# VITA-Group/Open-L2O

Measured on NVIDIA H100. Metric: coordinate-updates/sec (N_params x unroll_steps), higher is better.
Workload: dtype f32

## Files before the change

open_l2o_b200/csrc/cwlstm_tc.cuh:

```cuda
#pragma once
#include "cwlstm_common.cuh"
#include "l2o_internal.h"

namespace l2o {
namespace tc {

constexpr int kH = 20;
constexpr int kN = 4 * kH;
constexpr int kTile = 64;
constexpr int kU = 5;
constexpr int kFwdWG = 3;
constexpr int kFwdThreads = 128 * kFwdWG;
template <int N>
struct IC {
  static constexpr int value = N;
};

template <class C>
struct Geo {
  static constexpr bool FC = C::FC;
  static constexpr int ColH1 = FC ? 24 : 4, ColH2 = FC ? 44 : 24;
  static constexpr int ColOne = FC ? 20 : C::F;
  static constexpr int KB = FC ? 8 : 6;
  static constexpr int L1Lo = 0, L1Hi = FC ? 6 : 3;
  static constexpr int L2Lo = FC ? 2 : 0, L2Hi = KB;
  static constexpr int K1 = 8 * (L1Hi - L1Lo), K2 = 8 * (L2Hi - L2Lo);
  static constexpr int N1 = FC ? 48 : 24, N2 = 48;
  static constexpr int B1Floats = K1 * kN, B2Floats = K2 * kN, T1Floats = kN * N1, T2Floats = kN * N2;
  static constexpr int FwdFloats = 2 * (B1Floats + B2Floats);
  static constexpr int AllFloats = FwdFloats + 2 * (T1Floats + T2Floats);
  static_assert(!FC || C::F == 20, "fc preprocessing: dim 20");
  static_assert(FC || C::F <= 3, "feature chunk: at most 3 features");
};
constexpr int kImgMaxFloats = Geo<Cfg<L2O_PRE_FC, 2, 20, 20, 20>>::AllFloats;

__device__ __forceinline__ uint32_t smem_u32(const void* p) { return (uint32_t)__cvta_generic_to_shared(p); }

__device__ __forceinline__ void mbar_init(uint64_t* bar, uint32_t count) {
  asm volatile("mbarrier.init.shared::cta.b64 [%0], %1;" ::"r"(smem_u32(bar)), "r"(count));
}
__device__ __forceinline__ void mbar_expect_tx(uint64_t* bar, uint32_t bytes) {
  asm volatile("mbarrier.arrive.expect_tx.shared::cta.b64 _, [%0], %1;" ::"r"(smem_u32(bar)), "r"(bytes) : "memory");
}
__device__ __forceinline__ void mbar_wait(uint64_t* bar, uint32_t parity) {
  asm volatile(
      "{\n\t"
      ".reg .pred p;\n\t"
      "WAIT_LOOP:\n\t"
      "mbarrier.try_wait.parity.shared::cta.b64 p, [%0], %1;\n\t"
      "@p bra WAIT_DONE;\n\t"
      "bra WAIT_LOOP;\n\t"
      "WAIT_DONE:\n\t"
      "}\n" ::"r"(smem_u32(bar)),
      "r"(parity)
      : "memory");
}
__device__ __forceinline__ void fence_barrier_init() { asm volatile("fence.mbarrier_init.release.cluster;" ::: "memory"); }
__device__ __forceinline__ void fence_proxy_async() { asm volatile("fence.proxy.async.shared::cta;" ::: "memory"); }
__device__ __forceinline__ void tma_bulk_g2s(void* dst, const void* src, uint32_t bytes, uint64_t* bar) {
  asm volatile("cp.async.bulk.shared::cluster.global.mbarrier::complete_tx::bytes [%0], [%1], %2, [%3];" ::"r"(
                   smem_u32(dst)),
               "l"(src), "r"(bytes), "r"(smem_u32(bar))
               : "memory");
}
__device__ __forceinline__ void stage_image(float* dst, const float* src, uint32_t bytes, uint64_t* bar) {
  if (threadIdx.x == 0) {
    mbar_expect_tx(bar, bytes);
    tma_bulk_g2s(dst, src, bytes, bar);
  }
  mbar_wait(bar, 0);
}

__device__ __forceinline__ void wg_fence() { asm volatile("wgmma.fence.sync.aligned;" ::: "memory"); }
__device__ __forceinline__ void wg_commit() { asm volatile("wgmma.commit_group.sync.aligned;" ::: "memory"); }
template <int N>
__device__ __forceinline__ void wg_wait() {
  asm volatile("wgmma.wait_group.sync.aligned %0;" ::"n"(N) : "memory");
}

__device__ __forceinline__ uint64_t make_desc(uint32_t saddr, uint32_t lbo, uint32_t sbo) {
  return (uint64_t)((saddr & 0x3FFFFu) >> 4) | ((uint64_t)(lbo >> 4) << 16) | ((uint64_t)(sbo >> 4) << 32);
}
__device__ __forceinline__ uint64_t img_desc(const float* p, int ncols) {
  return make_desc(smem_u32(p), (uint32_t)(ncols / 8) * 128u, 128u);
}
__host__ __device__ constexpr uint64_t img_kstep(int ncols) { return (uint64_t)((2 * (ncols / 8) * 128) >> 4); }

#define L2O_ACC8(b) "+f"(d[b]), "+f"(d[b + 1]), "+f"(d[b + 2]), "+f"(d[b + 3]), "+f"(d[b + 4]), "+f"(d[b + 5]), \
                    "+f"(d[b + 6]), "+f"(d[b + 7])
__device__ __forceinline__ void mma_rs_n80(float* d, const uint32_t* a, uint64_t b, uint32_t acc) {
  asm volatile(
      "{\n\t.reg .pred p;\n\tsetp.ne.b32 p, %45, 0;\n\t"
      "wgmma.mma_async.sync.aligned.m64n80k8.f32.tf32.tf32 "
      "{%0,%1,%2,%3,%4,%5,%6,%7,%8,%9,%10,%11,%12,%13,%14,%15,%16,%17,%18,%19,"
      "%20,%21,%22,%23,%24,%25,%26,%27,%28,%29,%30,%31,%32,%33,%34,%35,%36,%37,%38,%39}, "
      "{%40,%41,%42,%43}, %44, p, 1, 1;\n\t}\n"
      : L2O_ACC8(0), L2O_ACC8(8), L2O_ACC8(16), L2O_ACC8(24), L2O_ACC8(32)
      : "r"(a[0]), "r"(a[1]), "r"(a[2]), "r"(a[3]), "l"(b), "r"(acc));
}
__device__ __forceinline__ void mma_rs_n48(float* d, const uint32_t* a, uint64_t b, uint32_t acc) {
  asm volatile(
      "{\n\t.reg .pred p;\n\tsetp.ne.b32 p, %29, 0;\n\t"
      "wgmma.mma_async.sync.aligned.m64n48k8.f32.tf32.tf32 "
      "{%0,%1,%2,%3,%4,%5,%6,%7,%8,%9,%10,%11,%12,%13,%14,%15,%16,%17,%18,%19,%20,%21,%22,%23}, "
      "{%24,%25,%26,%27}, %28, p, 1, 1;\n\t}\n"
      : L2O_ACC8(0), L2O_ACC8(8), L2O_ACC8(16)
      : "r"(a[0]), "r"(a[1]), "r"(a[2]), "r"(a[3]), "l"(b), "r"(acc));
}
__device__ __forceinline__ void mma_rs_n24(float* d, const uint32_t* a, uint64_t b, uint32_t acc) {
  asm volatile(
      "{\n\t.reg .pred p;\n\tsetp.ne.b32 p, %17, 0;\n\t"
      "wgmma.mma_async.sync.aligned.m64n24k8.f32.tf32.tf32 "
      "{%0,%1,%2,%3,%4,%5,%6,%7,%8,%9,%10,%11}, "
      "{%12,%13,%14,%15}, %16, p, 1, 1;\n\t}\n"
      : L2O_ACC8(0), "+f"(d[8]), "+f"(d[9]), "+f"(d[10]), "+f"(d[11])
      : "r"(a[0]), "r"(a[1]), "r"(a[2]), "r"(a[3]), "l"(b), "r"(acc));
}
template <int N>
__device__ __forceinline__ void mma_rs(float* d, const uint32_t* a, uint64_t b, uint32_t acc) {
  static_assert(N == 80 || N == 48 || N == 24, "wgmma width");
  if constexpr (N == 80) mma_rs_n80(d, a, b, acc);
  else if constexpr (N == 48) mma_rs_n48(d, a, b, acc);
  else mma_rs_n24(d, a, b, acc);
}

__device__ __forceinline__ float to_tf32(float x) {
  uint32_t r;
  asm("cvt.rna.tf32.f32 %0, %1;" : "=r"(r) : "f"(x));
  return __uint_as_float(r);
}
__device__ __forceinline__ void split_tf32(float x, uint32_t& hi, uint32_t& lo) {
  hi = __float_as_uint(x) & 0xFFFFE000u;
  lo = __float_as_uint(x - __uint_as_float(hi));
}

__host__ __device__ constexpr int vec_unit(int c, int base) { return 5 * ((c - base) & 3) + ((c - base) >> 2); }
__host__ __device__ constexpr int unit_col(int u, int base) { return base + 4 * (u % 5) + u / 5; }
__host__ __device__ constexpr int gate_ref_col(int n) {
  return (2 * ((n >> 3) & 1) + (n & 1)) * kH + 5 * ((n & 7) >> 1) + (n >> 4);
}
__host__ __device__ constexpr int dx_gate_col(int k) { return (k & ~7) + 2 * (k & 3) + ((k >> 2) & 1); }
__host__ __device__ constexpr int dx_group(int c) { return c / 24; }
__host__ __device__ constexpr int dx_unit(int c) {
  return 2 * ((c % 24) >> 3) + (c & 1) >= 5 ? -1 : 5 * ((c & 7) >> 1) + 2 * ((c % 24) >> 3) + (c & 1);
}
__host__ __device__ constexpr int img_index(int k, int n, int ncols) {
  return ((k >> 2) * (ncols / 8) + (n >> 3)) * 32 + (n & 7) * 4 + (k & 3);
}

template <class C>
__device__ __forceinline__ float ext_weight(const float* __restrict__ theta, bool l2, int c, int n) {
  using G = Geo<C>;
  const int col = gate_ref_col(n);
  if (c == G::ColOne) return theta[(l2 ? C::O_B2 : C::O_B1) + col];
  const bool in_h1 = c >= G::ColH1 && c < G::ColH1 + kH, in_h2 = c >= G::ColH2 && c < G::ColH2 + kH;
  if (!l2) {
    if (in_h1) return theta[C::O_W1 + (C::F + vec_unit(c, G::ColH1)) * C::G1 + col];
    if (G::FC && c < kH) return theta[C::O_W1 + vec_unit(c, 0) * C::G1 + col];
    if (!G::FC && c < C::F) return theta[C::O_W1 + c * C::G1 + col];
    return 0.f;
  }
  if (in_h1) return theta[C::O_W2 + vec_unit(c, G::ColH1) * C::G2 + col];
  if (in_h2) return theta[C::O_W2 + (kH + vec_unit(c, G::ColH2)) * C::G2 + col];
  return 0.f;
}
constexpr float kLog2e = 1.4426950408889634f;
__host__ __device__ constexpr float gate_scale(int gate) { return gate == 1 ? -2.f * kLog2e : -kLog2e; }
constexpr int kGateF = 2;
__device__ __forceinline__ float sigmoid_scaled(float zs) { return rcp_approx(1.0f + ex2_approx(zs)); }
__device__ __forceinline__ float tanh_scaled(float zs) { return fmaf(2.0f, rcp_approx(1.0f + ex2_approx(zs)), -1.0f); }

template <class C>
__host__ __device__ constexpr int dx_operand_col(bool l2, int c) {
  using G = Geo<C>;
  return l2 ? unit_col(dx_unit(c), dx_group(c) == 0 ? G::ColH1 : G::ColH2)
            : unit_col(dx_unit(c), dx_group(c) == 0 ? G::ColH1 : 0);
}

template <class C>
__global__ void prep_weights_kernel(const float* __restrict__ theta, float* __restrict__ img, int with_transposed) {
  static_assert(C::H1 == kH && C::H2 == kH && (C::F <= 3 || C::FC), "tc engine: LSTM-20x2, F <= 3 or fc(20)");
  using G = Geo<C>;
  const int nb = (G::K1 + G::K2) * kN;
  const int nt = with_transposed ? kN * (G::N1 + G::N2) : 0;
  for (int e = blockIdx.x * blockDim.x + threadIdx.x; e < nb + nt; e += gridDim.x * blockDim.x) {
    float w;
    float* hi;
    int off, idx;
    if (e < nb) {
      const bool l2 = e >= G::K1 * kN;
      const int ee = l2 ? e - G::K1 * kN : e;
      const int k = ee / kN, n = ee % kN;
      const int c = 8 * (l2 ? G::L2Lo : G::L1Lo) + k, gate = gate_ref_col(n) / kH;
      w = ext_weight<C>(theta, l2, c, n);
      if (c == G::ColOne && gate == kGateF) w += 1.0f;
      w *= gate_scale(gate);
      hi = img + (l2 ? 2 * G::B1Floats : 0);
      off = l2 ? G::B2Floats : G::B1Floats;
      idx = img_index(k, n, kN);
    } else {
      const int e2 = e - nb;
      const bool l2 = e2 >= kN * G::N1;
      const int nc = l2 ? G::N2 : G::N1;
      const int ee = l2 ? e2 - kN * G::N1 : e2;
      const int k = ee / nc, n = ee % nc;
      w = dx_unit(n) < 0 ? 0.f : ext_weight<C>(theta, l2, dx_operand_col<C>(l2, n), dx_gate_col(k));
      hi = img + G::FwdFloats + (l2 ? 2 * G::T1Floats : 0);
      off = l2 ? G::T2Floats : G::T1Floats;
      idx = img_index(k, n, nc);
    }
    const float h = to_tf32(w);
    hi[idx] = h;
    hi[off + idx] = to_tf32(w - h);
  }
}

template <int KB>
struct Frag {
  uint32_t hi[KB][4], lo[KB][4];
  __device__ __forceinline__ void zero() {
#pragma unroll
    for (int k = 0; k < KB; ++k)
#pragma unroll
      for (int r = 0; r < 4; ++r) { hi[k][r] = 0u; lo[k][r] = 0u; }
  }
  __device__ __forceinline__ void put_at(int c, int rh, float v) {
    split_tf32(v, hi[c / 8][((c / 4) & 1) * 2 + rh], lo[c / 8][((c / 4) & 1) * 2 + rh]);
  }
  __device__ __forceinline__ float get_at(int c, int rh) const {
    return __uint_as_float(hi[c / 8][((c / 4) & 1) * 2 + rh]) + __uint_as_float(lo[c / 8][((c / 4) & 1) * 2 + rh]);
  }
  template <int COL>
  __device__ __forceinline__ void put(int rh, float v) {
    static_assert(COL % 4 == 0 && COL / 8 < KB, "fragment column");
    put_at(COL, rh, v);
  }
  template <int BASE>
  __device__ __forceinline__ void put_vec(int rh, const float* v) {
    static_assert(BASE % 4 == 0 && (BASE + 19) / 8 < KB, "fragment column");
#pragma unroll
    for (int s = 0; s < kU; ++s) put_at(BASE + 4 * s, rh, v[s]);
  }
};

template <int N, int KB, int LO, int HI>
__device__ __forceinline__ void mma3(float* d, const Frag<KB>& f, uint64_t bh, uint64_t bl) {
  constexpr uint64_t step = img_kstep(N);
#pragma unroll
  for (int kb = LO; kb < HI; ++kb) {
    const uint64_t o = (uint64_t)(kb - LO) * step;
    mma_rs<N>(d, f.lo[kb], bh + o, kb > LO ? 1u : 0u);
    mma_rs<N>(d, f.hi[kb], bl + o, 1u);
    mma_rs<N>(d, f.hi[kb], bh + o, 1u);
  }
}

__host__ __device__ constexpr int acc_idx(int s, int g, int rh) { return 4 * (2 * s + (g >> 1)) + 2 * rh + (g & 1); }

__device__ __forceinline__ void lstm_point_fwd(float zi, float zj, float zf, float zo, float& c, float& h) {
  const float Ei = ex2_approx(fminf(zi, 40.f));
  const float Ej = ex2_approx(fminf(zj, 40.f));
  const float Qf = 1.0f + ex2_approx(fminf(zf, 40.f));
  const float Pij = (1.0f + Ei) * (1.0f + Ej);
  const float cn = fmaf(c, Pij, (1.0f - Ej) * Qf) * rcp_approx(Pij * Qf);
  c = cn;
  const float Ec = ex2_approx(fminf(-2.f * kLog2e * cn, 63.f));
  const float Eo = ex2_approx(fminf(zo, 63.f));
  h = (1.0f - Ec) * rcp_approx((1.0f + Ec) * (1.0f + Eo));
}
__device__ __forceinline__ float elu_fast(float av) {
  const float em = ex2_approx(kLog2e * av) - 1.0f;
  const float ep = av * fmaf(av, fmaf(av, fmaf(av, 1.0f / 24.0f, 1.0f / 6.0f), 0.5f), 1.0f);
  return av > 0.f ? av : (av > -0.0625f ? ep : em);
}

__device__ __forceinline__ void load5(const float* __restrict__ p, int q, float* v) {
#pragma unroll
  for (int s = 0; s < kU; ++s) v[s] = p[5 * q + s];
}
__device__ __forceinline__ void store5(float* __restrict__ p, int q, const float* v) {
#pragma unroll
  for (int s = 0; s < kU; ++s) p[5 * q + s] = v[s];
}
__device__ __forceinline__ float quad_sum(float v) {
  v += __shfl_xor_sync(0xffffffffu, v, 1);
  return v + __shfl_xor_sync(0xffffffffu, v, 2);
}
__device__ __forceinline__ float from_row(float v, int lane, int rh) {
  return __shfl_sync(0xffffffffu, v, (lane & ~3) | rh);
}

struct FwdExtra {
  const int32_t* step_ptr;
  int32_t t_offset;
  float p_fixed;
};

template <class C>
struct SmemF {
  float img[Geo<C>::FwdFloats];
  float wo[kH + 4];
  float win[64];
  uint64_t wbar;
};
template <class C>
__host__ __device__ constexpr size_t adamc_offset() {
  return (sizeof(SmemF<C>) + 15) & ~(size_t)15;
}
template <class C>
__host__ __device__ constexpr size_t fwd_smem_bytes(int T) {
  return adamc_offset<C>() + (C::FC ? (size_t)T * 2 * sizeof(float) : 0);
}
__device__ __forceinline__ double warp_sum_pairs_d(double v) {
  v += __shfl_xor_sync(0xffffffffu, v, 16);
  v += __shfl_xor_sync(0xffffffffu, v, 8);
  v += __shfl_xor_sync(0xffffffffu, v, 4);
  return v + __shfl_xor_sync(0xffffffffu, v, 1);
}

template <class C, bool FAST = false, int OPT = L2O_OPT_NONE, bool CKPT = false>
__global__ void __launch_bounds__(kFwdThreads, 1) unroll_fwd_kernel(l2o_unroll_args a, NetRt rt, const float* __restrict__ img,
                                                                     float* __restrict__ state_out, FwdExtra ex) {
  static_assert(!FAST || (!C::FC && OPT != L2O_OPT_NONE), "the full-tile forward is the DM nets' with an optimizee");
  using G = Geo<C>;
  extern __shared__ __align__(128) unsigned char smem_raw[];
  SmemF<C>& S = *reinterpret_cast<SmemF<C>*>(smem_raw);
  const int T = a.T;
  const int64_t n = a.n;
  const bool in_kernel_opt = FAST || a.opt_kind != L2O_OPT_NONE;
  const int opt_kind = FAST ? OPT : a.opt_kind;
  const bool want_fx = in_kernel_opt && a.fx != nullptr;
  const bool adam_mode = C::NIN == 2 && a.m != nullptr;
  const bool has_ckpt = FAST ? CKPT : a.ckpt != nullptr;
  const bool has_grec = FAST ? CKPT : a.g_rec != nullptr;
  const bool tanh_out = !FAST && rt.tanh_output;
  const bool has_delta = !FAST && a.delta_seq != nullptr;
  const bool has_labels = !FAST && a.labels != nullptr;
  float* adamc = reinterpret_cast<float*>(smem_raw + adamc_offset<C>());

  if (threadIdx.x < kH) S.wo[threadIdx.x] = a.theta[C::O_WO + threadIdx.x];
  if (threadIdx.x == kH) S.wo[kH] = a.theta[C::O_BO];
  if constexpr (C::FC) {
    static_assert(!C::FC || C::NIN == 2, "fc nets here are RNNprop nets (two inputs)");
    if (threadIdx.x >= 32 && threadIdx.x < 92) S.win[threadIdx.x - 32] = a.theta[C::O_WIN + threadIdx.x - 32];
    if (adam_mode) {
      const int step0 = ex.step_ptr ? *ex.step_ptr + ex.t_offset : a.step0;
      for (int t = threadIdx.x; t < T; t += blockDim.x) {
        const float p = (ex.step_ptr == nullptr && ex.p_fixed > 0.f) ? ex.p_fixed : (float)(step0 + t);
        adamc[2 * t] = 1.0f - powf(a.beta1, p);
        adamc[2 * t + 1] = 1.0f - powf(a.beta2, p);
      }
    }
  }
  if (threadIdx.x == 0) {
    mbar_init(&S.wbar, 1);
    fence_barrier_init();
  }
  __syncthreads();
  stage_image(S.img, img, G::FwdFloats * 4, &S.wbar);

  const int wg = __shfl_sync(0xffffffffu, threadIdx.x >> 7, 0), warp = (threadIdx.x >> 5) & 3, lane = threadIdx.x & 31;
  const int g = lane >> 2, q = lane & 3, own = q & 1;
  const uint64_t b1h = img_desc(S.img, kN), b1l = img_desc(S.img + G::B1Floats, kN);
  const uint64_t b2h = img_desc(S.img + 2 * G::B1Floats, kN), b2l = img_desc(S.img + 2 * G::B1Floats + G::B2Floats, kN);
  const int64_t ntiles = (n + kTile - 1) / kTile;
  const int64_t slot = n * C::SF;
  const int64_t nk = n * kH;
  const float bo = S.wo[kH];
  float wo[kU];
#pragma unroll
  for (int s = 0; s < kU; ++s) wo[s] = S.wo[5 * q + s];
  double imit = 0.0;
  float d[kN / 2];
#pragma unroll
  for (int k = 0; k < kN / 2; ++k) d[k] = 0.f;

  for (int64_t tile = (int64_t)blockIdx.x * kFwdWG + wg; tile < ntiles; tile += (int64_t)gridDim.x * kFwdWG) {
    const int64_t r0 = tile * kTile + warp * 16 + g;
    const int64_t row[2] = {r0, r0 + 8};
    const bool act[2] = {FAST || row[0] < n, FAST || row[1] < n};
    const int64_t io = own ? row[1] : row[0];
    const bool oact = FAST || io < n;
    const bool writer = q < 2 && oact;
    float* ck = has_ckpt ? a.ckpt + r0 * kH : nullptr;
    float* gr = has_grec ? a.g_rec + io : nullptr;
    Frag<G::KB> A;
    A.zero();
    float c1[2][kU], c2[2][kU];
#pragma unroll
    for (int rh = 0; rh < 2; ++rh) {
      float h1[kU] = {0.f, 0.f, 0.f, 0.f, 0.f}, h2[kU] = {0.f, 0.f, 0.f, 0.f, 0.f};
#pragma unroll
      for (int s = 0; s < kU; ++s) { c1[rh][s] = 0.f; c2[rh][s] = 0.f; }
      if (act[rh]) {
        const int64_t i = row[rh];
        load5(a.state + i * kH, q, h1);
        load5(a.state + (n + i) * kH, q, c1[rh]);
        load5(a.state + 2 * n * kH + i * kH, q, h2);
        load5(a.state + 2 * n * kH + (n + i) * kH, q, c2[rh]);
        if (has_ckpt) {
          float* p = ck + rh * 8 * kH;
          store5(p, q, h1);
          store5(p + nk, q, c1[rh]);
          store5(p + 2 * nk, q, h2);
          store5(p + 3 * nk, q, c2[rh]);
        }
        if (!FAST && T == 0 && state_out != a.state) {
          store5(state_out + i * kH, q, h1);
          store5(state_out + (n + i) * kH, q, c1[rh]);
          store5(state_out + 2 * n * kH + i * kH, q, h2);
          store5(state_out + 2 * n * kH + (n + i) * kH, q, c2[rh]);
        }
      }
      A.template put_vec<G::ColH1>(rh, h1);
      A.template put_vec<G::ColH2>(rh, h2);
    }
    if constexpr (G::FC) {
      A.template put<G::ColOne>(0, q == 0 ? 1.0f : 0.f);
      A.template put<G::ColOne>(1, q == 0 ? 1.0f : 0.f);
    }
    float x = 0.f, oa = 0.f, ob = 0.f, am = 0.f, av = 0.f;
    if (oact) {
      if (FAST || a.x) x = a.x[io];
      if (in_kernel_opt) { oa = a.opt_a[io]; ob = a.opt_b[io]; }
      if (adam_mode) { am = a.m[io]; av = a.v[io]; }
    }
// ... 193 lines not shown
```

open_l2o_b200/csrc/cwlstm_tc_bwd.cuh:

```cuda
#pragma once
#include <type_traits>
#include "cwlstm_tc.cuh"

namespace l2o {
namespace tcb {

using namespace tc;

constexpr int kBwdWG = 2;
constexpr int kBwdThreads = 128 * kBwdWG;
constexpr uint32_t kXaLBO = 8 * 128;
constexpr uint32_t kXbLBO = 10 * 128;
constexpr uint32_t kXaBytes = 8 * kXaLBO;
constexpr uint32_t kXbBytes = 8 * kXbLBO;
constexpr int kBlkL1 = 5, kRowOne2 = 63;

__device__ __forceinline__ void split_bf16x2(float v0, float v1, uint32_t& hi, uint32_t& lo) {
  asm("cvt.rn.bf16x2.f32 %0, %1, %2;" : "=r"(hi) : "f"(v1), "f"(v0));
  const float r0 = v0 - __uint_as_float(hi << 16), r1 = v1 - __uint_as_float(hi & 0xFFFF0000u);
  asm("cvt.rn.bf16x2.f32 %0, %1, %2;" : "=r"(lo) : "f"(r1), "f"(r0));
}
__device__ __forceinline__ void stsm_x4_trans(uint32_t sa, uint32_t r0, uint32_t r1, uint32_t r2, uint32_t r3) {
  asm volatile("stmatrix.sync.aligned.m8n8.x4.trans.shared.b16 [%0], {%1, %2, %3, %4};" ::"r"(sa), "r"(r0), "r"(r1),
               "r"(r2), "r"(r3)
               : "memory");
}
__device__ __forceinline__ void mma_ss_bf16_n80(float* d, uint64_t a, uint64_t b) {
  asm volatile(
      "{\n\t.reg .pred p;\n\tsetp.ne.b32 p, %42, 0;\n\t"
      "wgmma.mma_async.sync.aligned.m64n80k16.f32.bf16.bf16 "
      "{%0,%1,%2,%3,%4,%5,%6,%7,%8,%9,%10,%11,%12,%13,%14,%15,%16,%17,%18,%19,"
      "%20,%21,%22,%23,%24,%25,%26,%27,%28,%29,%30,%31,%32,%33,%34,%35,%36,%37,%38,%39}, "
      "%40, %41, p, 1, 1, 0, 0;\n\t}\n"
      : L2O_ACC8(0), L2O_ACC8(8), L2O_ACC8(16), L2O_ACC8(24), L2O_ACC8(32)
      : "l"(a), "l"(b), "r"(1));
}
__device__ __forceinline__ void wg_bar(int wg) { asm volatile("bar.sync %0, 128;" ::"r"(1 + wg) : "memory"); }
__device__ __forceinline__ void prefetch_l2_bulk(const void* p, uint32_t bytes) {
  asm volatile("cp.async.bulk.prefetch.L2.global [%0], %1;" ::"l"(p), "r"(bytes) : "memory");
}
__device__ __forceinline__ void prefetch_l2(const void* p) { asm volatile("prefetch.global.L2 [%0];" ::"l"(p)); }

__device__ __forceinline__ void unit_bwd(float& zi, float& zj, float& zf, float& zo, float cprev, float dh, float& dc, float& hn) {
  const float i = sigmoid_scaled(zi), j = tanh_scaled(zj), f = sigmoid_scaled(zf), o = sigmoid_scaled(zo);
  const float cn = fmaf(f, cprev, i * j);
  const float tcn = tanh_fast(cn);
  hn = tcn * o;
  const float dho = dh * o;
  const float dcv = fmaf(dho, fmaf(-tcn, tcn, 1.0f), dc);
  zi = (dcv * j) * fmaf(-i, i, i);
  zj = (dcv * i) * fmaf(-j, j, 1.0f);
  zf = (dcv * cprev) * fmaf(-f, f, f);
  zo = (dho * tcn) * (1.0f - o);
  dc = dcv * f;
}

template <class C, int MODE>
__device__ __forceinline__ int dw_row(int m) {
  const int p = (m & 7) >> 1, slot = 2 * (m >> 3) + (m & 1);
  if (m == kRowOne2) return MODE == 2 ? C::O_B1 : C::O_B2;
  if (slot < 2 * kBlkL1) {
    const int u = 5 * p + slot % kU;
    if (MODE == 2) return C::O_W1 + (slot < kU ? C::F + u : u) * C::G1;
    return C::O_W2 + (slot < kU ? u : kH + u) * C::G2;
  }
  if (MODE == 0) {
    const int s = slot - 2 * kBlkL1;
    if (s < kU) return C::O_W1 + (C::F + 5 * p + s) * C::G1;
    if (p < C::F) return C::O_W1 + p * C::G1;
    if (p == C::F) return C::O_B1;
  }
  return -1;
}

template <class C, int MODE>
struct SmemB {
  float img[Geo<C>::AllFloats];
  float wo[kH + 4];
  float win[64];
  uint64_t wbar, pad;
};
template <class C, int MODE>
__host__ __device__ constexpr uint32_t stage_bytes() {
  return (MODE == 0 ? 4 : 2) * kXaBytes + 2 * kXbBytes;
}
struct alignas(16) CkRing {
  float h[tc::kTile * kH], c2[tc::kTile * kH], c1[tc::kTile * kH];
  uint64_t barh, bar2, bar1;
};
template <class C, int MODE>
__host__ __device__ constexpr size_t bwd_smem_bytes() {
  return ((sizeof(SmemB<C, MODE>) + 1023) & ~(size_t)1023) +
         (size_t)kBwdWG * (stage_bytes<C, MODE>() + (MODE == 0 ? sizeof(CkRing) : 0));
}

constexpr int kFlImit = 1, kFlTanh = 2;

template <class C, int MODE, bool CARRY, int FL, bool FULL>
__global__ void __launch_bounds__(kBwdThreads, 1) unroll_bwd_kernel(l2o_bwd_args a, NetRt rt, const float* __restrict__ img,
                                                                    l2o_bwd_carry cy) {
  using G = Geo<C>;
  static_assert(MODE == 0 ? !C::FC : C::FC, "DM nets: one pass; fc nets: two passes");
  static_assert(MODE != 0 || C::F < 3, "the feature chunk leaves quad thread 3's slot of row 63 to layer 2's 1");
  static_assert(MODE != 2 || FL == 0, "the output-layer flags belong to the layer-2 passes");
  static_assert(MODE == 0 || !FULL, "the full-tile body is the DM nets'");
  constexpr bool kImit = (FL & kFlImit) != 0, kTanh = (FL & kFlTanh) != 0;
  extern __shared__ __align__(1024) unsigned char smem_raw[];
  SmemB<C, MODE>& S = *reinterpret_cast<SmemB<C, MODE>*>(smem_raw);
  const int wg = __shfl_sync(0xffffffffu, threadIdx.x >> 7, 0);
  const int warp = (threadIdx.x >> 5) & 3, lane = threadIdx.x & 31;
  const int g = lane >> 2, q = lane & 3;
  const uint32_t stage = smem_u32(smem_raw) + (uint32_t)((sizeof(SmemB<C, MODE>) + 1023) & ~(size_t)1023) +
                         (uint32_t)wg * stage_bytes<C, MODE>();
  constexpr uint32_t kXa2 = 0, kXa1 = 2 * kXaBytes;
  constexpr uint32_t kXb = (MODE == 0 ? 4 : 2) * kXaBytes;
  constexpr bool kL2 = MODE != 2, kL1 = MODE != 1;
  constexpr bool kRing = MODE == 0;
  CkRing& R = *reinterpret_cast<CkRing*>(smem_raw + ((sizeof(SmemB<C, MODE>) + 1023) & ~(size_t)1023) +
                                         (size_t)kBwdWG * stage_bytes<C, MODE>() + (size_t)wg * sizeof(CkRing));
  const bool elected = (threadIdx.x & 127) == 0;

  for (uint32_t o = threadIdx.x * 4; o < kBwdWG * stage_bytes<C, MODE>(); o += blockDim.x * 4) {
    const uint32_t ow = o % stage_bytes<C, MODE>();
    const uint32_t v = (ow < kXaBytes && (ow % kXaLBO) >> 4 == (uint32_t)kRowOne2) ? 0x3F803F80u : 0u;
    asm volatile("st.shared.u32 [%0], %1;" ::"r"(stage - (uint32_t)wg * stage_bytes<C, MODE>() + o), "r"(v) : "memory");
  }
  if (threadIdx.x < kH) S.wo[threadIdx.x] = a.theta[C::O_WO + threadIdx.x];
  if constexpr (C::FC) {
    if (threadIdx.x >= 32 && threadIdx.x < 92) S.win[threadIdx.x - 32] = a.theta[C::O_WIN + threadIdx.x - 32];
  }
  if (threadIdx.x == 0) {
    mbar_init(&S.wbar, 1);
    if (!kRing) fence_barrier_init();
  }
  if (kRing && elected) {
    mbar_init(&R.barh, 1);
    mbar_init(&R.bar2, 1);
    mbar_init(&R.bar1, 1);
    fence_barrier_init();
  }
  fence_proxy_async();
  __syncthreads();
  stage_image(S.img, img, G::AllFloats * 4, &S.wbar);

  const uint64_t b1h = img_desc(S.img, kN), b1l = img_desc(S.img + G::B1Floats, kN);
  const uint64_t b2h = img_desc(S.img + 2 * G::B1Floats, kN), b2l = img_desc(S.img + 2 * G::B1Floats + G::B2Floats, kN);
  const float* tbase = S.img + G::FwdFloats;
  const uint64_t t1h = img_desc(tbase, G::N1), t1l = img_desc(tbase + G::T1Floats, G::N1);
  const uint64_t t2h = img_desc(tbase + 2 * G::T1Floats, G::N2), t2l = img_desc(tbase + 2 * G::T1Floats + G::T2Floats, G::N2);
  const uint64_t xbh = make_desc(stage + kXb, kXbLBO, 128), xbl = make_desc(stage + kXb + kXbBytes, kXbLBO, 128);
  const uint64_t xa2h = make_desc(stage + kXa2, kXaLBO, 128), xa2l = make_desc(stage + kXa2 + kXaBytes, kXaLBO, 128);
  const uint64_t xa1h = make_desc(stage + (MODE == 0 ? kXa1 : kXa2), kXaLBO, 128);
  const uint64_t xa1l = make_desc(stage + (MODE == 0 ? kXa1 : kXa2) + kXaBytes, kXaLBO, 128);

  const int T = a.T;
  const int64_t n = a.n, slot = n * C::SF;
  const int64_t ntiles = (n + tc::kTile - 1) / tc::kTile;
  const float inv_nt = kImit ? 1.0f / (float)a.n_total : 0.f;
  float wo[kU];
#pragma unroll
  for (int s = 0; s < kU; ++s) wo[s] = S.wo[5 * q + s];
  float acc_wo[kU] = {0.f, 0.f, 0.f, 0.f, 0.f}, acc_bo = 0.f;
  float aw0[kU] = {0.f, 0.f, 0.f, 0.f, 0.f}, aw1[kU] = {0.f, 0.f, 0.f, 0.f, 0.f}, ab[kU] = {0.f, 0.f, 0.f, 0.f, 0.f};
  float dw[kN / 2];
#pragma unroll
  for (int k = 0; k < kN / 2; ++k) dw[k] = 0.f;
  const int kx = warp * 16 + g;
  const int64_t tstride = (int64_t)gridDim.x * kBwdWG;
  const int64_t nkh = n * kH;
  const int64_t ck_wrap = (int64_t)(T - 1) * slot + tstride * tc::kTile * kH;

  auto ck_block = [&](const float* ckt, int blk) {
    return ckt + blk * nkh;
  };
  auto tile_bytes = [&](int64_t tl) {
    const int64_t r = n - tl * tc::kTile;
    return (uint32_t)((r < tc::kTile ? r : tc::kTile) * kH * 4);
  };
  auto arm = [&](uint64_t* bar, float* dst, const float* ckt, int blk, uint32_t b) {
    mbar_expect_tx(bar, b);
    tma_bulk_g2s(dst, ck_block(ckt, blk), b, bar);
  };
  auto ring5 = [&](const float* buf, int rh, bool on, float* v) {
    const float* p = buf + (kx + 8 * rh) * kH + 5 * q;
#pragma unroll
    for (int s = 0; s < kU; ++s) v[s] = on ? p[s] : 0.f;
  };
  if constexpr (kRing) {
    const int64_t tile0 = (int64_t)blockIdx.x * kBwdWG + wg;
    if (elected && tile0 < ntiles) {
      const float* ck0 = a.ckpt + (int64_t)(T - 1) * slot + tile0 * tc::kTile * kH;
      const uint32_t b = tile_bytes(tile0);
      arm(&R.barh, R.h, ck0, 2, b);
      arm(&R.bar2, R.c2, ck0, 3, b);
      arm(&R.bar1, R.c1, ck0, 1, b);
    }
  }
  uint32_t ph = 0;

  Frag<G::KB> A;
  const int blk = lane >> 3;
  const uint32_t la = stage + (uint32_t)((2 * warp + (blk & 1)) * (int)kXaLBO + (blk >> 1) * (int)kXaBytes + (lane & 7) * 16);
  const uint32_t lb = stage + kXb + (uint32_t)((2 * warp + (blk & 1)) * (int)kXbLBO + (blk >> 1) * (int)kXbBytes + (lane & 7) * 16);
  auto stage_x = [&](uint32_t buf, int b0, int nb, int c0, int c1) {
    auto val = [&](int i, int rh) { return A.get_at(i < kU ? c0 + 4 * i : c1 + 4 * (i - kU), rh); };
#pragma unroll
    for (int b = 0; b < nb; ++b) {
      uint32_t h0, l0, h1, l1;
      split_bf16x2(val(2 * b, 0), val(2 * b + 1, 0), h0, l0);
      split_bf16x2(val(2 * b, 1), val(2 * b + 1, 1), h1, l1);
      stsm_x4_trans(la + buf + (uint32_t)(b0 + b) * 128, h0, h1, l0, l1);
    }
  };
  auto stage_dz = [&](const float* z) {
#pragma unroll
    for (int j = 0; j < kN / 8; ++j) {
      uint32_t h0, l0, h1, l1;
      split_bf16x2(z[4 * j], z[4 * j + 1], h0, l0);
      split_bf16x2(z[4 * j + 2], z[4 * j + 3], h1, l1);
      stsm_x4_trans(lb + (uint32_t)j * 128, h0, h1, l0, l1);
    }
  };
  auto dx_dw = [&](auto ncols, float* z, float* x, uint64_t th, uint64_t tl, uint64_t xah, uint64_t xal) {
    constexpr int NX = decltype(ncols)::value;
    uint32_t fh[kN / 8][4], fl[kN / 8][4];
#pragma unroll
    for (int j = 0; j < kN / 8; ++j) {
      split_tf32(z[4 * j + 0], fh[j][0], fl[j][0]);
      split_tf32(z[4 * j + 2], fh[j][1], fl[j][1]);
      split_tf32(z[4 * j + 1], fh[j][2], fl[j][2]);
      split_tf32(z[4 * j + 3], fh[j][3], fl[j][3]);
    }
    constexpr uint64_t step = img_kstep(NX);
    wg_fence();
#pragma unroll
    for (int j = 0; j < kN / 8; ++j) {
      mma_rs<NX>(x, fl[j], th + j * step, j > 0 ? 1u : 0u);
      mma_rs<NX>(x, fh[j], tl + j * step, 1u);
      mma_rs<NX>(x, fh[j], th + j * step, 1u);
    }
    wg_commit();
    constexpr uint64_t sa = (2 * kXaLBO) >> 4, sb = (2 * kXbLBO) >> 4;
#pragma unroll
    for (int kk = 0; kk < tc::kTile / 16; ++kk) {
      mma_ss_bf16_n80(dw, xal + kk * sa, xbh + kk * sb);
      mma_ss_bf16_n80(dw, xah + kk * sa, xbl + kk * sb);
      mma_ss_bf16_n80(dw, xah + kk * sa, xbh + kk * sb);
    }
    wg_commit();
    wg_wait<1>();
  };
  auto flush_dw = [&]() {
    wg_wait<0>();
#pragma unroll
    for (int rh = 0; rh < 2; ++rh) {
      const int r = dw_row<C, MODE>(kx + 8 * rh);
#pragma unroll
      for (int j = 0; j < kN / 8; ++j)
#pragma unroll
        for (int e = 0; e < 2; ++e) {
          float& v = dw[4 * j + 2 * rh + e];
          if (r >= 0 && v != 0.f) atomicAdd(&a.dtheta[r + gate_ref_col(8 * j + 2 * q + e)], (double)v);
          v = 0.f;
        }
    }
  };

  for (int64_t tile = (int64_t)blockIdx.x * kBwdWG + wg; tile < ntiles; tile += tstride) {
    const int64_t r0 = tile * tc::kTile + kx;
    const int64_t row[2] = {r0, r0 + 8};
    const bool act[2] = {FULL || row[0] < n, FULL || row[1] < n};
    const float* ckt = a.ckpt + (int64_t)(T - 1) * slot + tile * tc::kTile * kH;
    int64_t tn = (int64_t)(T - 1) * n;
    float dc2[2][kU], dh2c[2][kU], dc1[2][kU], dh1c[2][kU];
#pragma unroll
    for (int rh = 0; rh < 2; ++rh)
#pragma unroll
      for (int s = 0; s < kU; ++s) { dc2[rh][s] = 0.f; dh2c[rh][s] = 0.f; dc1[rh][s] = 0.f; dh1c[rh][s] = 0.f; }
    float lam[2];
#pragma unroll
    for (int rh = 0; rh < 2; ++rh) lam[rh] = (kL2 && act[rh] && !kImit) ? a.g_rec[tn + n + row[rh]] : 0.f;
    if constexpr (CARRY) {
#pragma unroll
      for (int rh = 0; rh < 2; ++rh) {
        if (!act[rh]) continue;
        const int64_t i = row[rh];
        if constexpr (kL2) {
          load5(cy.d_state + (2 * n + i) * kH, q, dh2c[rh]);
          load5(cy.d_state + (3 * n + i) * kH, q, dc2[rh]);
          lam[rh] = cy.lam[i] + a.g_rec[tn + n + i];
        }
        if constexpr (kL1) {
          load5(cy.d_state + i * kH, q, dh1c[rh]);
          load5(cy.d_state + (n + i) * kH, q, dc1[rh]);
        }
      }
    }
    A.zero();
    A.template put<(G::ColOne & ~3)>(0, q == (G::ColOne & 3) ? 1.0f : 0.f);
    A.template put<(G::ColOne & ~3)>(1, q == (G::ColOne & 3) ? 1.0f : 0.f);

    for (int t = T - 1; t >= 0; --t) {
      const float* ckr = ckt + kx * kH;
      float z[kN / 2];
      float dh1n[2][kU];
      if constexpr (kL2) {
        float c2p[2][kU], dy[2];
        if constexpr (kRing) mbar_wait(&R.barh, 0);
#pragma unroll
        for (int rh = 0; rh < 2; ++rh) {
          float h1n[kU] = {0.f, 0.f, 0.f, 0.f, 0.f}, h2p[kU] = {0.f, 0.f, 0.f, 0.f, 0.f};
#pragma unroll
          for (int s = 0; s < kU; ++s) c2p[rh][s] = 0.f;
          float dtanh = 1.0f;
          if (act[rh]) {
            const float* cr = ckr + 8 * kH * rh;
            if constexpr (kRing) {
              if (t == T - 1) load5(cr + slot, q, h1n);
              ring5(R.h, rh, true, h2p);
            } else {
              load5(cr + slot, q, h1n);
              load5(cr + 2 * nkh, q, h2p);
              load5(cr + 3 * nkh, q, c2p[rh]);
            }
            if constexpr (kImit) lam[rh] = (a.delta_seq[tn + row[rh]] - a.labels[tn + row[rh]]) * inv_nt;
            if constexpr (kTanh) {
              const float th = a.delta_seq[tn + row[rh]] / rt.scale;
              dtanh = fmaf(-th, th, 1.0f);
            }
          }
          dy[rh] = rt.scale * lam[rh] * dtanh;
          if (!kRing || t == T - 1) A.template put_vec<G::ColH1>(rh, h1n);
          A.template put_vec<G::ColH2>(rh, h2p);
        }
        wg_fence();
        mma3<kN, G::KB, G::L2Lo, G::L2Hi>(z, A, b2h, b2l);
        wg_commit();
        wg_wait<0>();
        if constexpr (kRing) {
          mbar_wait(&R.bar2, ph);
#pragma unroll
          for (int rh = 0; rh < 2; ++rh) ring5(R.c2, rh, act[rh], c2p[rh]);
        }
        if (q == 0) acc_bo += dy[0] + dy[1];
#pragma unroll
        for (int rh = 0; rh < 2; ++rh)
#pragma unroll
          for (int s = 0; s < kU; ++s) {
            float hn;
            unit_bwd(z[acc_idx(s, 0, rh)], z[acc_idx(s, 1, rh)], z[acc_idx(s, 2, rh)], z[acc_idx(s, 3, rh)], c2p[rh][s],
                     fmaf(wo[s], dy[rh], dh2c[rh][s]), dc2[rh][s], hn);
            acc_wo[s] = fmaf(hn, dy[rh], acc_wo[s]);
          }
        wg_bar(wg);
        if constexpr (kRing) {
          if (elected) {
            const int64_t tl_next = t > 0 ? tile : tile + tstride;
            arm(&R.barh, R.h, ckt, 0, tile_bytes(tile));
            if (tl_next < ntiles) arm(&R.bar2, R.c2, t > 0 ? ckt - slot : ckt + ck_wrap, 3, tile_bytes(tl_next));
          }
        }
        stage_x(kXa2, 0, kBlkL1, G::ColH1, G::ColH2);
        stage_dz(z);
        fence_proxy_async();
        wg_bar(wg);
        float x2[G::N2 / 2];
        dx_dw(IC<G::N2>{}, z, x2, t2h, t2l, xa2h, xa2l);
#pragma unroll
        for (int rh = 0; rh < 2; ++rh)
#pragma unroll
          for (int s = 0; s < kU; ++s) {
            dh1n[rh][s] = x2[4 * (s >> 1) + 2 * rh + (s & 1)];
            dh2c[rh][s] = x2[4 * (3 + (s >> 1)) + 2 * rh + (s & 1)];
          }
        if constexpr (MODE == 1) {
#pragma unroll
          for (int rh = 0; rh < 2; ++rh)
            if (act[rh]) store5(a.scratch + (tn + row[rh]) * kH, q, dh1n[rh]);
        }
#pragma unroll
        for (int rh = 0; rh < 2; ++rh)
          if (!kImit && act[rh] && (!CARRY || t > 0)) lam[rh] += a.g_rec[tn + row[rh]];
      }
      if constexpr (kL1) {
        float c1p[2][kU];
        float r0v[2] = {0.f, 0.f};
        [[maybe_unused]] float r1v[2] = {0.f, 0.f};
        [[maybe_unused]] float ep[2][kU];
        if constexpr (kRing) mbar_wait(&R.barh, 1);
#pragma unroll
        for (int rh = 0; rh < 2; ++rh) {
          float h1p[kU] = {0.f, 0.f, 0.f, 0.f, 0.f};
#pragma unroll
          for (int s = 0; s < kU; ++s) c1p[rh][s] = 0.f;
          if (act[rh]) {
            if constexpr (kRing) {
              ring5(R.h, rh, true, h1p);
            } else {
              load5(ckr + 8 * kH * rh, q, h1p);
              load5(ckr + nkh + 8 * kH * rh, q, c1p[rh]);
            }
            if constexpr (MODE == 2) {
              load5(a.scratch + (tn + row[rh]) * kH, q, dh1n[rh]);
              r0v[rh] = a.in_seq[2 * tn + row[rh]];
              r1v[rh] = a.in_seq[2 * tn + n + row[rh]];
            } else {
              r0v[rh] = a.in_seq[tn + row[rh]];
            }
          } else if constexpr (MODE == 2) {
#pragma unroll
            for (int s = 0; s < kU; ++s) dh1n[rh][s] = 0.f;
          }
          A.template put_vec<G::ColH1>(rh, h1p);
          if constexpr (MODE == 2) {
            float e[kU];
#pragma unroll
            for (int s = 0; s < kU; ++s) {
              const int u = 5 * q + s;
              const float av = fmaf(r1v[rh], S.win[kH + u], fmaf(r0v[rh], S.win[u], S.win[2 * kH + u]));
              e[s] = elu_fast(av);
              ep[rh][s] = av > 0.f ? 1.0f : e[s] + 1.0f;
            }
            A.template put_vec<0>(rh, e);
          } else {
            float f[C::F];
            preprocess<C>(nullptr, rt, r0v[rh], 0.f, f);
            float v = q == C::F ? 1.0f : 0.f;
#pragma unroll
            for (int k = 0; k < C::F; ++k)
              if (q == k) v = f[k];
            A.template put<0>(rh, v);
          }
        }
        wg_fence();
        mma3<kN, G::KB, G::L1Lo, G::L1Hi>(z, A, b1h, b1l);
        wg_commit();
        wg_wait<0>();
        if constexpr (kRing) {
          mbar_wait(&R.bar1, ph);
#pragma unroll
          for (int rh = 0; rh < 2; ++rh) ring5(R.c1, rh, act[rh], c1p[rh]);
        }
#pragma unroll
        for (int rh = 0; rh < 2; ++rh)
#pragma unroll
          for (int s = 0; s < kU; ++s) {
            float hn;
            unit_bwd(z[acc_idx(s, 0, rh)], z[acc_idx(s, 1, rh)], z[acc_idx(s, 2, rh)], z[acc_idx(s, 3, rh)], c1p[rh][s],
                     dh1c[rh][s] + dh1n[rh][s], dc1[rh][s], hn);
          }
        wg_bar(wg);
        if constexpr (kRing) {
          const int64_t tl_next = t > 0 ? tile : tile + tstride;
          if (elected && tl_next < ntiles) {
            const float* ckn = t > 0 ? ckt - slot : ckt + ck_wrap;
            const uint32_t b = tile_bytes(tl_next);
            arm(&R.barh, R.h, ckn, 2, b);
            arm(&R.bar1, R.c1, ckn, 1, b);
            prefetch_l2_bulk(ck_block(ckn, 0), b);
          }
          const int64_t rn = t > 0 ? r0 : r0 + tstride * tc::kTile;
          const float* in_next = a.in_seq + (t > 0 ? tn - n : (int64_t)(T - 1) * n) + rn;
#pragma unroll
          for (int rh = 0; rh < 2; ++rh)
            if (q == 0 && ((FULL && t > 0) || rn + 8 * rh < n)) prefetch_l2(in_next + 8 * rh);
          ph ^= 1u;
        }
        if constexpr (MODE == 2) stage_x(kXa2, 0, kBlkL1, G::ColH1, 0);
        else stage_x(kXa1, kBlkL1, 3, G::ColH1, 0);
        stage_dz(z);
        fence_proxy_async();
        wg_bar(wg);
        float x1[G::N1 / 2];
        dx_dw(IC<G::N1>{}, z, x1, t1h, t1l, xa1h, xa1l);
#pragma unroll
        for (int rh = 0; rh < 2; ++rh)
#pragma unroll
          for (int s = 0; s < kU; ++s) {
            dh1c[rh][s] = x1[4 * (s >> 1) + 2 * rh + (s & 1)];
            if constexpr (MODE == 2) {
              const float da = x1[4 * (3 + (s >> 1)) + 2 * rh + (s & 1)] * ep[rh][s];
              aw0[s] = fmaf(r0v[rh], da, aw0[s]);
              aw1[s] = fmaf(r1v[rh], da, aw1[s]);
              ab[s] += da;
            }
          }
      }
      ckt -= slot;
      tn -= n;
    }
    if constexpr (CARRY) {
#pragma unroll
      for (int rh = 0; rh < 2; ++rh) {
        if (!act[rh]) continue;
        const int64_t i = row[rh];
        if constexpr (kL2) {
          store5(cy.d_state + (2 * n + i) * kH, q, dh2c[rh]);
          store5(cy.d_state + (3 * n + i) * kH, q, dc2[rh]);
          if (q == 0) cy.lam[i] = lam[rh];
        }
        if constexpr (kL1) {
          store5(cy.d_state + i * kH, q, dh1c[rh]);
          store5(cy.d_state + (n + i) * kH, q, dc1[rh]);
        }
      }
    }
    flush_dw();
  }
  wg_wait<0>();
  auto red8 = [&](float v) {
#pragma unroll
    for (int o = 4; o < 32; o <<= 1) v += __shfl_xor_sync(0xffffffffu, v, o);
    return v;
  };
#pragma unroll
  for (int s = 0; s < kU; ++s) {
    const int u = 5 * q + s;
    if constexpr (kL2) {
      const float v = red8(acc_wo[s]);
      if (lane < 4) atomicAdd(&a.dtheta[C::O_WO + u], (double)v);
    }
    if constexpr (MODE == 2) {
      const float v0 = red8(aw0[s]), v1 = red8(aw1[s]), vb = red8(ab[s]);
      if (lane < 4) {
        atomicAdd(&a.dtheta[C::O_WIN + u], (double)v0);
        atomicAdd(&a.dtheta[C::O_WIN + C::F + u], (double)v1);
        atomicAdd(&a.dtheta[C::O_BIN + u], (double)vb);
      }
    }
  }
  if constexpr (kL2) {
    const float v = red8(acc_bo);
    if (lane == 0) atomicAdd(&a.dtheta[C::O_BO], (double)v);
  }
}

}

template <class C, bool CARRY>
int tc_launch_bwd(const char* fn, const NetRt& rt, const l2o_bwd_args& a, float* img, cudaStream_t st, int sms,
                  const l2o_bwd_carry& cy) {
  tc::prep_weights_kernel<C><<<16, 256, 0, st>>>(a.theta, img, 1);
  if (int rc = after_launch(fn)) return rc;
  const int64_t ntiles = (a.n + tc::kTile - 1) / tc::kTile;
  const int64_t ctas = (ntiles + tcb::kBwdWG - 1) / tcb::kBwdWG;
  const int grid = (int)(ctas < sms ? ctas : sms);
  auto launch = [&](auto kern, size_t smem) {
    if (smem > 227 * 1024) return L2O_E_INVALID;
    if (int rc = raise_smem_limit(fn, kern, smem)) return rc;
    kern<<<grid, tcb::kBwdThreads, smem, st>>>(a, rt, img, cy);
    return after_launch(fn);
  };
  const int fl = (a.labels != nullptr ? tcb::kFlImit : 0) | (rt.tanh_output ? tcb::kFlTanh : 0);
  auto launch_l2 = [&](auto mode, auto full) {
    constexpr int M = decltype(mode)::value;
    constexpr bool F = decltype(full)::value;
    constexpr size_t smem = tcb::bwd_smem_bytes<C, M>();
    switch (fl) {
      case 0: return launch(tcb::unroll_bwd_kernel<C, M, CARRY, 0, F>, smem);
      case tcb::kFlImit: return launch(tcb::unroll_bwd_kernel<C, M, CARRY, tcb::kFlImit, F>, smem);
      case tcb::kFlTanh: return launch(tcb::unroll_bwd_kernel<C, M, CARRY, tcb::kFlTanh, F>, smem);
      default: return launch(tcb::unroll_bwd_kernel<C, M, CARRY, tcb::kFlImit | tcb::kFlTanh, F>, smem);
    }
  };
  if constexpr (C::FC) {
    int rc = launch_l2(tc::IC<1>{}, std::false_type{});
    if (rc != L2O_OK) return rc;
    return launch(tcb::unroll_bwd_kernel<C, 2, CARRY, 0, false>, tcb::bwd_smem_bytes<C, 2>());
  } else {
    if (a.n % tc::kTile == 0) return launch_l2(tc::IC<0>{}, std::true_type{});
    return launch_l2(tc::IC<0>{}, std::false_type{});
  }
}

}
```

Before: 1.985 billion.

## Use scaled f16 split-precision wgmma for 48-column backward dX products

For the 48-column dX products in the backward kernel, the transposed weight images are converted once per block into power-of-two-scaled f16 hi/lo pairs in shared memory. The per-row gate gradients are rescaled the same way and split into f16 hi/lo, so k16 f16 wgmmas replace k8 tf32 wgmmas, halving the number of MMA instructions over K. Results are unscaled afterwards. This adds a per-block max reduction and conversion pass at startup and per-call shuffles for scaling, and it risks precision loss from f16's narrow exponent range, which the scaling is meant to contain.

```diff
diff --git a/open_l2o_b200/csrc/cwlstm_tc.cuh b/open_l2o_b200/csrc/cwlstm_tc.cuh
--- a/open_l2o_b200/csrc/cwlstm_tc.cuh
+++ b/open_l2o_b200/csrc/cwlstm_tc.cuh
@@ -81,7 +81,7 @@
 __device__ __forceinline__ uint64_t make_desc(uint32_t saddr, uint32_t lbo, uint32_t sbo) {
   return (uint64_t)((saddr & 0x3FFFFu) >> 4) | ((uint64_t)(lbo >> 4) << 16) | ((uint64_t)(sbo >> 4) << 32);
 }
-__device__ __forceinline__ uint64_t img_desc(const float* p, int ncols) {
+__device__ __forceinline__ uint64_t img_desc(const void* p, int ncols) {
   return make_desc(smem_u32(p), (uint32_t)(ncols / 8) * 128u, 128u);
 }
 __host__ __device__ constexpr uint64_t img_kstep(int ncols) { return (uint64_t)((2 * (ncols / 8) * 128) >> 4); }
@@ -122,6 +122,15 @@
   if constexpr (N == 80) mma_rs_n80(d, a, b, acc);
   else if constexpr (N == 48) mma_rs_n48(d, a, b, acc);
   else mma_rs_n24(d, a, b, acc);
+}
+__device__ __forceinline__ void mma_rs_f16_n48(float* d, const uint32_t* a, uint64_t b, uint32_t acc) {
+  asm volatile(
+      "{\n\t.reg .pred p;\n\tsetp.ne.b32 p, %29, 0;\n\t"
+      "wgmma.mma_async.sync.aligned.m64n48k16.f32.f16.f16 "
+      "{%0,%1,%2,%3,%4,%5,%6,%7,%8,%9,%10,%11,%12,%13,%14,%15,%16,%17,%18,%19,%20,%21,%22,%23}, "
+      "{%24,%25,%26,%27}, %28, p, 1, 1, 0;\n\t}\n"
+      : L2O_ACC8(0), L2O_ACC8(8), L2O_ACC8(16)
+      : "r"(a[0]), "r"(a[1]), "r"(a[2]), "r"(a[3]), "l"(b), "r"(acc));
 }
 
 __device__ __forceinline__ float to_tf32(float x) {
diff --git a/open_l2o_b200/csrc/cwlstm_tc_bwd.cuh b/open_l2o_b200/csrc/cwlstm_tc_bwd.cuh
--- a/open_l2o_b200/csrc/cwlstm_tc_bwd.cuh
+++ b/open_l2o_b200/csrc/cwlstm_tc_bwd.cuh
@@ -73,13 +73,84 @@
   return -1;
 }
 
+__host__ __device__ constexpr bool dx_f16(int ncols) { return ncols == 48; }
+template <class C>
+struct BwdImg {
+  using G = Geo<C>;
+  static constexpr bool F16L1 = dx_f16(G::N1);
+  static_assert(dx_f16(G::N2), "layer 2's dX is 48 columns wide");
+  static constexpr int TmaFloats = G::FwdFloats + (F16L1 ? 0 : 2 * G::T1Floats);
+  static constexpr int T2Word = F16L1 ? G::T1Floats : 0;
+  static constexpr int Words = T2Word + G::T2Floats;
+};
+
+__device__ __forceinline__ uint32_t f16x2_rz(float v0, float v1) {
+  uint32_t r;
+  asm("cvt.rz.f16x2.f32 %0, %1, %2;" : "=r"(r) : "f"(v1), "f"(v0));
+  return r;
+}
+__device__ __forceinline__ void split_f16x2(float v0, float v1, uint32_t& hi, uint32_t& lo) {
+  uint32_t h0, l0, h1, l1;
+  split_tf32(v0, h0, l0);
+  split_tf32(v1, h1, l1);
+  hi = f16x2_rz(__uint_as_float(h0), __uint_as_float(h1));
+  lo = f16x2_rz(__uint_as_float(l0), __uint_as_float(l1));
+}
+__device__ __forceinline__ int f16_scale_exp(float m) { return 141 - (int)(__float_as_uint(m) >> 23); }
+__device__ __forceinline__ float exp2_int(int e) { return __int_as_float((e + 127) << 23); }
+
 template <class C, int MODE>
 struct SmemB {
-  float img[Geo<C>::AllFloats];
+  float img[BwdImg<C>::TmaFloats];
+  uint32_t timg[BwdImg<C>::Words];
   float wo[kH + 4];
   float win[64];
+  float wmax[kBwdThreads / 32][2];
+  int tsc[2];
   uint64_t wbar, pad;
 };
+
+template <class C, int MODE>
+__device__ __forceinline__ void stage_dx_images(SmemB<C, MODE>& S, const float* __restrict__ src) {
+  using G = Geo<C>;
+  using I = BwdImg<C>;
+  auto finite_abs = [](float v) { return fabsf(v) < INFINITY ? fabsf(v) : 0.f; };
+  float m[2] = {0.f, 0.f};
+  if (I::F16L1)
+    for (int i = threadIdx.x; i < G::T1Floats; i += blockDim.x) m[0] = fmaxf(m[0], finite_abs(src[i]));
+  for (int i = threadIdx.x; i < G::T2Floats; i += blockDim.x) m[1] = fmaxf(m[1], finite_abs(src[2 * G::T1Floats + i]));
+#pragma unroll
+  for (int l = 0; l < 2; ++l) {
+#pragma unroll
+    for (int o = 1; o < 32; o <<= 1) m[l] = fmaxf(m[l], __shfl_xor_sync(0xffffffffu, m[l], o));
+    if ((threadIdx.x & 31) == 0) S.wmax[threadIdx.x >> 5][l] = m[l];
+  }
+  __syncthreads();
+  int sc[2];
+#pragma unroll
+  for (int l = 0; l < 2; ++l) {
+    float mm = 0.f;
+#pragma unroll
+    for (int w = 0; w < kBwdThreads / 32; ++w) mm = fmaxf(mm, S.wmax[w][l]);
+    sc[l] = min(f16_scale_exp(mm), 127);
+  }
+  if (threadIdx.x == 0) { S.tsc[0] = sc[0]; S.tsc[1] = sc[1]; }
+  constexpr int P1 = I::F16L1 ? G::T1Floats / 2 : 0, P2 = G::T2Floats / 2;
+  for (int e = threadIdx.x; e < 2 * (P1 + P2); e += blockDim.x) {
+    const bool l2 = e >= 2 * P1;
+    const int nc = l2 ? G::N2 : G::N1, np = l2 ? P2 : P1;
+    const int ee = l2 ? e - 2 * P1 : e;
+    const bool lo = ee >= np;
+    const int w = lo ? ee - np : ee;
+    const int p = w & 3, blk = w >> 5, kb = blk / (nc / 8), n = 8 * (blk % (nc / 8)) + ((w >> 2) & 7);
+    const float* t = src + (l2 ? 2 * G::T1Floats : 0) + (lo ? (l2 ? G::T2Floats : G::T1Floats) : 0);
+    const float s = exp2_int(sc[l2]);
+    S.timg[(l2 ? I::T2Word : 0) + (lo ? np : 0) + w] =
+        f16x2_rz(t[img_index(8 * kb + p, n, nc)] * s, t[img_index(8 * kb + 4 + p, n, nc)] * s);
+  }
+  fence_proxy_async();
+  __syncthreads();
+}
 template <class C, int MODE>
 __host__ __device__ constexpr uint32_t stage_bytes() {
   return (MODE == 0 ? 4 : 2) * kXaBytes + 2 * kXbBytes;
@@ -141,13 +212,16 @@
   }
   fence_proxy_async();
   __syncthreads();
-  stage_image(S.img, img, G::AllFloats * 4, &S.wbar);
+  stage_dx_images(S, img + G::FwdFloats);
+  stage_image(S.img, img, BwdImg<C>::TmaFloats * 4, &S.wbar);
 
   const uint64_t b1h = img_desc(S.img, kN), b1l = img_desc(S.img + G::B1Floats, kN);
   const uint64_t b2h = img_desc(S.img + 2 * G::B1Floats, kN), b2l = img_desc(S.img + 2 * G::B1Floats + G::B2Floats, kN);
-  const float* tbase = S.img + G::FwdFloats;
-  const uint64_t t1h = img_desc(tbase, G::N1), t1l = img_desc(tbase + G::T1Floats, G::N1);
-  const uint64_t t2h = img_desc(tbase + 2 * G::T1Floats, G::N2), t2l = img_desc(tbase + 2 * G::T1Floats + G::T2Floats, G::N2);
+  const uint64_t t1h = BwdImg<C>::F16L1 ? img_desc(S.timg, G::N1) : img_desc(S.img + G::FwdFloats, G::N1);
+  const uint64_t t1l = BwdImg<C>::F16L1 ? img_desc(S.timg + G::T1Floats / 2, G::N1)
+                                        : img_desc(S.img + G::FwdFloats + G::T1Floats, G::N1);
+  const uint64_t t2h = img_desc(S.timg + BwdImg<C>::T2Word, G::N2);
+  const uint64_t t2l = img_desc(S.timg + BwdImg<C>::T2Word + G::T2Floats / 2, G::N2);
   const uint64_t xbh = make_desc(stage + kXb, kXbLBO, 128), xbl = make_desc(stage + kXb + kXbBytes, kXbLBO, 128);
   const uint64_t xa2h = make_desc(stage + kXa2, kXaLBO, 128), xa2l = make_desc(stage + kXa2 + kXaBytes, kXaLBO, 128);
   const uint64_t xa1h = make_desc(stage + (MODE == 0 ? kXa1 : kXa2), kXaLBO, 128);
@@ -221,23 +295,59 @@
       stsm_x4_trans(lb + (uint32_t)j * 128, h0, h1, l0, l1);
     }
   };
-  auto dx_dw = [&](auto ncols, float* z, float* x, uint64_t th, uint64_t tl, uint64_t xah, uint64_t xal) {
+  auto dx_dw = [&](auto ncols, float* z, float* x, int s, uint64_t th, uint64_t tl, uint64_t xah, uint64_t xal) {
     constexpr int NX = decltype(ncols)::value;
-    uint32_t fh[kN / 8][4], fl[kN / 8][4];
-#pragma unroll
-    for (int j = 0; j < kN / 8; ++j) {
-      split_tf32(z[4 * j + 0], fh[j][0], fl[j][0]);
-      split_tf32(z[4 * j + 2], fh[j][1], fl[j][1]);
-      split_tf32(z[4 * j + 1], fh[j][2], fl[j][2]);
-      split_tf32(z[4 * j + 3], fh[j][3], fl[j][3]);
-    }
-    constexpr uint64_t step = img_kstep(NX);
-    wg_fence();
-#pragma unroll
-    for (int j = 0; j < kN / 8; ++j) {
-      mma_rs<NX>(x, fl[j], th + j * step, j > 0 ? 1u : 0u);
-      mma_rs<NX>(x, fh[j], tl + j * step, 1u);
-      mma_rs<NX>(x, fh[j], th + j * step, 1u);
+    [[maybe_unused]] float un[2];
+    if constexpr (dx_f16(NX)) {
+      const int elo = max(-126, -127 - s), ehi = min(127, 126 - s);
+      float sc[2];
+#pragma unroll
+      for (int rh = 0; rh < 2; ++rh) {
+        float v[kN / 8];
+#pragma unroll
+        for (int j = 0; j < kN / 8; ++j) v[j] = fmaxf(fabsf(z[4 * j + 2 * rh]), fabsf(z[4 * j + 2 * rh + 1]));
+#pragma unroll
+        for (int w = 1; w < kN / 8; w <<= 1)
+#pragma unroll
+          for (int j = 0; j + w < kN / 8; j += 2 * w) v[j] = fmaxf(v[j], v[j + w]);
+        float m = v[0];
+        m = fmaxf(m, __shfl_xor_sync(0xffffffffu, m, 1));
+        m = fmaxf(m, __shfl_xor_sync(0xffffffffu, m, 2));
+        const int e = min(max(f16_scale_exp(m), elo), ehi);
+        sc[rh] = exp2_int(e);
+        un[rh] = exp2_int(-e - s);
+      }
+      uint32_t fh[kN / 16][4], fl[kN / 16][4];
+#pragma unroll
+      for (int m = 0; m < kN / 16; ++m)
+#pragma unroll
+        for (int r = 0; r < 4; ++r)
+          split_f16x2(z[8 * m + 2 * r] * sc[r & 1], z[8 * m + 2 * r + 1] * sc[r & 1], fh[m][r], fl[m][r]);
+      constexpr uint64_t step = img_kstep(NX);
+      wg_fence();
+#pragma unroll
+      for (int m = 0; m < kN / 16; ++m) {
+        mma_rs_f16_n48(x, fl[m], th + m * step, m > 0 ? 1u : 0u);
+        mma_rs_f16_n48(x, fh[m], tl + m * step, 1u);
+        mma_rs_f16_n48(x, fh[m], th + m * step, 1u);
+      }
+    } else {
+      uint32_t fh[kN / 8][4], fl[kN / 8][4];
+#pragma unroll
+      for (int j = 0; j < kN / 8; ++j) {
+        split_tf32(z[4 * j + 0], fh[j][0], fl[j][0]);
+        split_tf32(z[4 * j + 2], fh[j][1], fl[j][1]);
+        split_tf32(z[4 * j + 1], fh[j][2], fl[j][2]);
+        split_tf32(z[4 * j + 3], fh[j][3], fl[j][3]);
+      }
+      constexpr uint64_t step = img_kstep(NX);
+      wg_fence();
+#pragma unroll
+      for (int j = 0; j < kN / 8; ++j) {
+        mma_rs<NX>(x, fl[j], th + j * step, j > 0 ? 1u : 0u);
+        mma_rs<NX>(x, fh[j], tl + j * step, 1u);
+        mma_rs<NX>(x, fh[j], th + j * step, 1u);
+      }
     }
     wg_commit();
     constexpr uint64_t sa = (2 * kXaLBO) >> 4, sb = (2 * kXbLBO) >> 4;
@@ -249,6 +359,10 @@
     }
     wg_commit();
     wg_wait<1>();
+    if constexpr (dx_f16(NX)) {
+#pragma unroll
+      for (int i = 0; i < NX / 2; ++i) x[i] *= un[(i >> 1) & 1];
+    }
   };
   auto flush_dw = [&]() {
     wg_wait<0>();
@@ -365,7 +479,7 @@
         fence_proxy_async();
         wg_bar(wg);
         float x2[G::N2 / 2];
-        dx_dw(IC<G::N2>{}, z, x2, t2h, t2l, xa2h, xa2l);
+        dx_dw(IC<G::N2>{}, z, x2, S.tsc[1], t2h, t2l, xa2h, xa2l);
 #pragma unroll
         for (int rh = 0; rh < 2; ++rh)
 #pragma unroll
@@ -472,7 +586,7 @@
         fence_proxy_async();
         wg_bar(wg);
         float x1[G::N1 / 2];
-        dx_dw(IC<G::N1>{}, z, x1, t1h, t1l, xa1h, xa1l);
+        dx_dw(IC<G::N1>{}, z, x1, S.tsc[0], t1h, t1l, xa1h, xa1l);
 #pragma unroll
         for (int rh = 0; rh < 2; ++rh)
 #pragma unroll
```

Measured after the change: 1.986 billion (median of 6 runs). About the same (+0.1%).
